# zharmad/SpinRelax

Measured on AMD Instinct MI355X. Metric: frame-vector-lag triples/s, C(t) + fit + R1/R2/NOE pipeline, higher is better.
Workload: dtype f32 transforms + f64 mean terms and chunk statistics (C(t): the reference's own type); f64 (histogram, fit, J(w), R1/R2/NOE)

## Files before the change

spinrelax_amd/csrc/sr_ct32.hip:

```cpp
#include "sr_internal.h"
#include "sr_ct32_fft.h"

namespace {

#ifndef SR_CT32_PF
#define SR_CT32_PF 0
#endif
#ifndef SR_CT32_NT
#define SR_CT32_NT 2
#endif
#ifndef SR_CT32_WAVES16
#define SR_CT32_WAVES16 3
#endif
#ifndef SR_CT32_WAVES
#define SR_CT32_WAVES 4
#endif
template <int N1, bool FULL>
__global__ __launch_bounds__(256, (N1 == 16 ? SR_CT32_WAVES16 : SR_CT32_WAVES)) void k_ct_rfft32(Ct32Args a)
{
    extern __shared__ __align__(16) unsigned char f32_smem[];
    c32 *lds = reinterpret_cast<c32 *>(f32_smem);
    constexpr int H = N1 * 256, M = 2 * H;
    constexpr int NZ = N1 == 4 ? 3 : (N1 == 8 ? 6 : (N1 == 12 ? 8 : 16));
    constexpr int IPT = N1 == 4 ? 3 : (N1 == 8 ? 6 : (N1 == 12 ? 8 : 11));
    c32 *tw1 = lds + rfft_img_slots(N1) + 256;
    c32 *tw3 = tw1 + 1024;
    float *aux = reinterpret_cast<float *>(tw3 + 256);
    const int tid0 = threadIdx.x;
    const int v = blockIdx.x / a.R, r = blockIdx.x - v * a.R;
    const int F = FULL ? 512 * NZ : a.F, L = FULL ? 256 * NZ : a.L;
    const int64_t start = a.chunk_start ? a.chunk_start[r] : (int64_t)r * F;
#ifdef SR_CT32_EXP_HOTLOADS
    const float *px = a.soa + (start & 1);
#else
    const float *px = a.soa + ((int64_t)v * 3 + 0) * a.Npad + start;
#endif
    const bool even = FULL || ((start | a.Npad | (int64_t)F) & 1) == 0;

#define SR_F32_LOAD1(DST, PLANE, T) SR_F32_LOADP(DST, PLANE, T, 0, NZ, 0)
#define SR_F32_LOADR(DST, PLANE, T, LO, HI) SR_F32_LOADP(DST, PLANE, T, LO, HI, 0)
#define SR_F32_LOAD1NT(DST, PLANE, T) SR_F32_LOADP(DST, PLANE, T, 0, NZ, SR_CT32_NT)
#define SR_F32_LOADP(DST, PLANE, T, LO, HI, POL)                                                 \
    {                                                                                            \
        const __amdgpu_buffer_rsrc_t rs_ = __builtin_amdgcn_make_buffer_rsrc(                    \
            const_cast<float *>(px + (int64_t)__builtin_amdgcn_readfirstlane(PLANE) * a.Npad), (short)0, F * 4, 0x00020000); \
        if (even) {                                                                              \
            _Pragma("unroll") for (int n1 = (LO); n1 < (HI); ++n1)                              \
                DST[n1] = __builtin_bit_cast(c32, __builtin_amdgcn_raw_buffer_load_b64(rs_, 8 * ((T) + 256 * n1), 0, (POL))); \
        } else {                                                                                 \
            _Pragma("unroll") for (int n1 = (LO); n1 < (HI); ++n1) {                            \
                const int ob_ = 8 * ((T) + 256 * n1);                                            \
                DST[n1] = c32{__builtin_bit_cast(float, __builtin_amdgcn_raw_buffer_load_b32(rs_, ob_, 0, (POL))),           \
                              __builtin_bit_cast(float, __builtin_amdgcn_raw_buffer_load_b32(rs_, ob_ + 4, 0, (POL)))};      \
            }                                                                                    \
        }                                                                                        \
    }
#define SR_F32_MASK(D0, D1, T, N1_)                                                              \
    if (!FULL) {                                                                                 \
        D0 = 2 * ((T) + 256 * (N1_)) < F ? D0 : 0.f;                                             \
        D1 = 2 * ((T) + 256 * (N1_)) + 1 < F ? D1 : 0.f;                                         \
    }
    {
        const int j = ((tid0 & 15) * (tid0 >> 4)) & 255;
        lds[rfft_img_slots(N1) + tid0] = c32{a.tab->w2[2 * j], a.tab->w2[2 * j + 1]};
#pragma unroll
        for (int jj = 0; jj < 4; ++jj) tw1[256 * jj + tid0] = c32{a.tab->w1[jj][2 * tid0], a.tab->w1[jj][2 * tid0 + 1]};
        tw3[tid0] = c32{a.tab->w3[2 * tid0], a.tab->w3[2 * tid0 + 1]};
        if (tid0 == 0) aux[50] = 0.f;
    }

    c32 sig[N1];
#pragma unroll
    for (int n1 = 0; n1 < N1; ++n1) sig[n1] = c32{0.f, 0.f};
    int nsig;
    {
        c32 xr[NZ], yr[NZ], zr[NZ];
        SR_F32_LOAD1(xr, 0, tid0)
        SR_F32_LOAD1(yr, 1, tid0)
        SR_F32_LOAD1NT(zr, 2, tid0)
        c32 s0 = {0.f, 0.f}, s1 = s0, s2 = s0, s3 = s0, s4 = s0, s5 = s0;
        float emax = 0.f;
#pragma unroll
        for (int n1 = 0; n1 < NZ; ++n1) {
            const c32 x = xr[n1], y = yr[n1], z = zr[n1];
            const c32 xx = x * x, yy = y * y, zz = z * z, q = xx + yy;
            s0 += (zz + zz) - q;
            s1 += xx - yy;
            s2 = pk_fma(x, y, s2);
            s3 = pk_fma(x, z, s3);
            s4 = pk_fma(y, z, s4);
            s5 += q + zz;
            c32 ev = (q + zz) - splat(1.0f);
            SR_F32_MASK(ev.x, ev.y, tid0, n1)
            emax = fmaxf(emax, fmaxf(fabsf(ev.x), fabsf(ev.y)));
        }
        const float t0 = wave_total_f32(s0.x + s0.y), t1 = wave_total_f32(s1.x + s1.y), t2 = wave_total_f32(s2.x + s2.y);
        const float t3 = wave_total_f32(s3.x + s3.y), t4 = wave_total_f32(s4.x + s4.y), t5 = wave_total_f32(s5.x + s5.y);
        emax = wave_max_f32(emax);
        if ((tid0 & 63) == 63) {
            float *o = aux + 8 * (tid0 >> 6);
            o[0] = t0; o[1] = t1; o[2] = t2; o[3] = t3; o[4] = t4; o[5] = t5; o[6] = emax;
        }
        __syncthreads();
        float m[6];
        const float invF = 1.0f / (float)F;
#pragma unroll
        for (int c = 0; c < 6; ++c)
            m[c] = __builtin_bit_cast(float, __builtin_amdgcn_readfirstlane(
                       __builtin_bit_cast(int, ((aux[c] + aux[8 + c]) + (aux[16 + c] + aux[24 + c])) * invF) & (int)0xFFFFFFF0));
        const float mx = fmaxf(fmaxf(aux[6], aux[14]), fmaxf(aux[22], aux[30]));
        const bool unit = __builtin_amdgcn_readfirstlane(mx < kUnitTolF ? 1 : 0) != 0;
        nsig = unit ? 5 : 6;
        const float wgt[6] = {1.0f, 3.0f, 12.0f, 12.0f, 12.0f, 2.0f};
        double Kc = unit ? 2.0 : 0.0;
#pragma unroll
        for (int c = 0; c < 6; ++c)
            if (c < 5 || !unit) Kc = fma((double)wgt[c] * (double)m[c], (double)m[c], Kc);
        if (tid0 == 0) {
#pragma unroll
            for (int c = 0; c < 6; ++c) {
                aux[32 + c] = m[c];
                aux[40 + c] = wgt[c] * m[c];
            }
            aux[48] = unit ? 2.0f : 0.f;
            *reinterpret_cast<double *>(aux + 52) = Kc;
        }
#pragma unroll
        for (int n1 = 0; n1 < NZ; ++n1) {
            c32 d = f32_sig0(xr[n1], yr[n1], zr[n1], m[0]);
            SR_F32_MASK(d.x, d.y, tid0, n1)
            sig[n1] = d;
        }
    }
    c32 W2[8];
#pragma unroll
    for (int q = 0; q < 8; ++q) W2[q] = c32{0.f, 0.f};
#ifdef SR_CT32_STAMPS
    long long stamp_acc[12] = {0, 0, 0, 0, 0, 0, 0, 0, 0, 0, 0, 0}, stamp_t = __builtin_amdgcn_s_memtime();
    const long long stamp_begin = stamp_t;
#define SR_STAMP_ARGS , stamp_acc, stamp_t
#else
#define SR_STAMP_ARGS
#endif
#pragma unroll 1
    for (int c = 0; c < nsig; ++c) {
        asm volatile("" ::: "memory");
        const int tid = opaque(tid0);
        const int k1 = (tid >> 4) & 15, k2a = tid & 15;
        const bool act = k1 < N1;
        const int pt = k1 != 0 ? (N1 - k1) * 16 + (15 - k2a) : (k2a != 0 ? 16 - k2a : 0);
        const int off0 = tid == 0 ? 1 : 0;
        const int cn = c + 1;
        c32 ar[NZ], br[NZ];
        if (SR_CT32_PF == 1 && cn < nsig) {
            SR_F32_LOAD1(ar, f32_plane_a(cn), tid)
            SR_F32_LOAD1(br, f32_plane_b(cn), tid)
        }
        c32 w[16];
        rfft32_workgroup<N1, true>(sig, w, lds, tw1, tid SR_STAMP_ARGS);
        SR_STAMP(6)
        if (SR_CT32_PF == 2 && cn < nsig) {
            SR_F32_LOAD1(ar, f32_plane_a(cn), tid)
            SR_F32_LOAD1(br, f32_plane_b(cn), tid)
        }
        SR_CT32_SYNC();
        SR_STAMP(7)
        if (act) {
            const float wgt = c == 0 ? 0.25f : (c == 1 ? 0.75f : (c == 5 ? 0.5f : 3.0f));
            const c32 *b = lds + 17 * pt + off0;
            const c32 wb = tw3[k1 + N1 * k2a];
#pragma unroll
            for (int q = 0; q < 8; q += 2) {
                const c32 zk0 = w[bitrev<4>(q)], zm0 = b[15 - q], zk1 = w[bitrev<4>(q + 1)], zm1 = b[14 - q];
                const c32 S0 = add_conj(zk0, zm0), S1 = add_conj(zk1, zm1);
                c32 T0 = sub_conj(zk0, zm0), T1 = sub_conj(zk1, zm1);
                cmulf2(T0, mulf_w32_rt(wb, q), T1, mulf_w32_rt(wb, q + 1));
                const c32 A0 = pair_re(S0, T0), B0 = pair_im(S0, T0), A1 = pair_re(S1, T1), B1 = pair_im(S1, T1);
                W2[q] = pk_fma(splat(wgt), pk_fma(A0, A0, B0 * B0), W2[q]);
                W2[q + 1] = pk_fma(splat(wgt), pk_fma(A1, A1, B1 * B1), W2[q + 1]);
            }
            if (off0) {
                const c32 zk = w[bitrev<4>(8)];
                const c32 D = {0.0f, 2.0f * zk.y};
                const c32 T = cmulf(D, mulf_w32_rt(wb, 8));
                const float pr = 2.0f * zk.x + T.y, pi = -T.x;
                aux[50] = fmaf(wgt, fmaf(pr, pr, pi * pi), aux[50]);
            }
        }
        SR_STAMP(8)
        if (cn < nsig) {
            asm volatile("" ::: "memory");
            const float mc = __builtin_bit_cast(float, __builtin_amdgcn_readfirstlane(__builtin_bit_cast(int, aux[32 + cn])));
#pragma unroll
            for (int g0 = 0; g0 < NZ; g0 += 8) {
                constexpr int GE = 8 < NZ ? 8 : NZ;
                if (g0 > 0) asm volatile("" ::: "memory");
                if (SR_CT32_PF == 0 || g0 > 0) {
                    if (SR_CT32_NT != 0 && cn == 3) {
                        SR_F32_LOADP(ar, 0, tid, g0, g0 + GE, SR_CT32_NT)
                    } else {
                        SR_F32_LOADR(ar, f32_plane_a(cn), tid, g0, g0 + GE)
                    }
                    if (SR_CT32_NT != 0 && cn == 2) {
                        SR_F32_LOADP(br, 1, tid, g0, g0 + GE, SR_CT32_NT)
                    } else {
                        SR_F32_LOADR(br, f32_plane_b(cn), tid, g0, g0 + GE)
                    }
                }
                if (cn == 1) {
#pragma unroll
                    for (int n1 = g0; n1 < g0 + GE; ++n1) ar[n1] = f32_sig1(ar[n1], br[n1], mc);
                } else if (cn == 5) {
                    c32 zr[NZ];
                    SR_F32_LOADR(zr, 2, tid, g0, g0 + GE)
#pragma unroll
                    for (int n1 = g0; n1 < g0 + GE; ++n1) ar[n1] = f32_sig5(ar[n1], br[n1], zr[n1], mc);
                } else {
#pragma unroll
                    for (int n1 = g0; n1 < g0 + GE; ++n1) ar[n1] = f32_sigp(ar[n1], br[n1], mc);
                }
#pragma unroll
                for (int n1 = g0; n1 < g0 + GE; ++n1) {
                    c32 d = ar[n1];
                    SR_F32_MASK(d.x, d.y, tid, n1)
                    sig[n1] = d;
                }
            }
#pragma unroll
            for (int n1 = NZ; n1 < N1; ++n1) sig[n1] = c32{0.f, 0.f};
        }
        SR_STAMP(9)
        SR_CT32_SYNC();
        SR_STAMP(10)
    }
#ifdef SR_CT32_STAMPS
    const long long stamp_loop_end = stamp_t;
#endif

    const int tid = opaque(tid0);
    const int k1 = (tid >> 4) & 15, k2a = tid & 15;
    const bool act = k1 < N1;
    const int pt = k1 != 0 ? (N1 - k1) * 16 + (15 - k2a) : (k2a != 0 ? 16 - k2a : 0);
    const int off0 = tid == 0 ? 1 : 0;
    if (act) {
        c32 *bk = lds + k1 + (N1 + 1) * k2a;
        c32 *bm = lds + (pt >> 4) + (N1 + 1) * (pt & 15) + 16 * (N1 + 1) * off0;
        const c32 wb = tw3[k1 + N1 * k2a];
#pragma unroll
        for (int q = 0; q < 8; ++q) {
            const float E = W2[q].x + W2[q].y, d = W2[q].x - W2[q].y;
            const c32 wk = mulf_w32_rt(wb, q);
            bk[16 * (N1 + 1) * q] = c32{fmaf(d, wk.y, E), d * wk.x};
            if (!(q == 0 && off0)) bm[16 * (N1 + 1) * (15 - q)] = c32{fmaf(-d, wk.y, E), d * wk.x};
        }
        if (off0) bk[16 * (N1 + 1) * 8] = c32{2.0f * aux[50], 0.0f};
    }
    __syncthreads();
    c32 w[16];
    {
        c32 yin[N1];
#pragma unroll
        for (int n1 = 0; n1 < N1; ++n1) {
            const int k = tid + 256 * n1;
            yin[n1] = lds[k + k / N1];
        }
        __syncthreads();
        rfft32_workgroup<N1, false>(yin, w, lds, tw1, tid SR_STAMP_ARGS);
    }
    __syncthreads();

    float *E = reinterpret_cast<float *>(lds);
    double *Tt = reinterpret_cast<double *>(lds);
    double *tot = reinterpret_cast<double *>(aux);
    {
        c32 xr[NZ], yr[NZ], zr[NZ];
        SR_F32_LOAD1NT(xr, 0, tid)
        SR_F32_LOAD1NT(yr, 1, tid)
        SR_F32_LOAD1NT(zr, 2, tid)
        float mm[6], wm[6];
#pragma unroll
        for (int c = 0; c < 6; ++c) {
            mm[c] = __builtin_bit_cast(float, __builtin_amdgcn_readfirstlane(__builtin_bit_cast(int, aux[32 + c])));
            wm[c] = __builtin_bit_cast(float, __builtin_amdgcn_readfirstlane(__builtin_bit_cast(int, aux[40 + c])));
        }
        const float weps = __builtin_bit_cast(float, __builtin_amdgcn_readfirstlane(__builtin_bit_cast(int, aux[48])));
        const bool unit = nsig == 5;
#pragma unroll
        for (int n1 = 0; n1 < NZ; ++n1) {
            const c32 x = xr[n1], y = yr[n1], z = zr[n1];
            c32 acc;
            if (unit) {
                acc.x = weps * (float)fma((double)x.x, (double)x.x, fma((double)y.x, (double)y.x, fma((double)z.x, (double)z.x, -1.0)));
                acc.y = weps * (float)fma((double)x.y, (double)x.y, fma((double)y.y, (double)y.y, fma((double)z.y, (double)z.y, -1.0)));
            } else {
                acc = splat(wm[5]) * f32_sig5(x, y, z, mm[5]);
            }
            acc = pk_fma(splat(wm[0]), f32_sig0(x, y, z, mm[0]), acc);
            acc = pk_fma(splat(wm[1]), f32_sig1(x, y, mm[1]), acc);
            acc = pk_fma(splat(wm[2]), f32_sigp(x, y, mm[2]), acc);
            acc = pk_fma(splat(wm[3]), f32_sigp(x, z, mm[3]), acc);
            acc = pk_fma(splat(wm[4]), f32_sigp(y, z, mm[4]), acc);
            SR_F32_MASK(acc.x, acc.y, tid, n1)
            *reinterpret_cast<c32 *>(E + 2 * (tid + 256 * n1)) = acc;
        }
    }
    __syncthreads();
    const int i0 = IPT * (255 - tid);
    double sfx[IPT], incl;
    {
        double hsum[IPT];
#pragma unroll
        for (int k = 0; k < IPT; ++k) {
            const int i = i0 + k, j = F - 1 - i;
            const float ei = E[min(i, F - 1)], ej = E[max(j, 0)];
            hsum[k] = (i <= j ? (double)ei : 0.0) + (i < j ? (double)ej : 0.0);
        }
        sfx[IPT - 1] = hsum[IPT - 1];
#pragma unroll
        for (int k = IPT - 2; k >= 0; --k) sfx[k] = hsum[k] + sfx[k + 1];
        incl = wave_scan_f64(sfx[0]);
        if ((tid & 63) == 63) tot[tid >> 6] = incl;
    }
    __syncthreads();
    {
        const int wave = tid >> 6;
        double off = incl - sfx[0];
#pragma unroll
        for (int w2 = 0; w2 < 3; ++w2) off += w2 < wave ? tot[w2] : 0.0;
        const double G0 = (tot[0] + tot[1]) + (tot[2] + tot[3]);
        const double Kc = *reinterpret_cast<const double *>(aux + 52);
#pragma unroll
        for (int k = 0; k < IPT; ++k) {
            const int d = i0 + k;
            if (d <= L) Tt[d] = fma((double)(F - d), Kc, G0 + (sfx[k] + off));
        }
        if (tid == 0 && L >= 256 * IPT) Tt[L] = fma((double)(F - L), Kc, G0);
    }
    __syncthreads();
    if (act) {
        double *out = a.psum + ((int64_t)v * a.R + r) * a.Lp;
        const double inv = 1.0 / (double)M, sixth = 1.0 / 6.0;
#pragma unroll
        for (int p = 0; p < 16; ++p) {
            const int m = k1 + N1 * (k2a + 16 * bitrev<4>(p));
            const int le = 2 * m, lod = 2 * m - 1;
            if (le >= 1 && le <= L) out[le] = fma((double)w[p].x, inv, Tt[le]) * sixth;
            if (lod >= 1 && lod <= L) out[lod] = fma((double)w[p].y, inv, Tt[lod]) * sixth;
        }
    }
#ifdef SR_CT32_STAMPS
    if ((tid & 63) == 0) {
        double *dbg = a.psum + ((int64_t)v * a.R + r) * a.Lp + L + 2 + 16 * (tid >> 6);
        for (int i = 0; i < 11; ++i) dbg[i] = (double)stamp_acc[i];
        dbg[11] = (double)(stamp_loop_end - stamp_begin);
        dbg[12] = (double)(__builtin_amdgcn_s_memtime() - stamp_begin);
    }
#endif
#undef SR_F32_LOAD1
#undef SR_F32_LOAD1NT
#undef SR_F32_LOADR
#undef SR_F32_LOADP
#undef SR_F32_MASK
}

template <int N1>
constexpr size_t f32_lds_bytes()
{
    return (size_t)(rfft_img_slots(N1) + 256 + 1024 + 256) * sizeof(c32) + 64 * sizeof(float);
}

template <int N1, bool FULL>
int launch_ct_rfft32_h(sr_ctx *ctx, const Ct32Args &a, int64_t series)
{
    size_t lds = f32_lds_bytes<N1>();
    static_assert(f32_lds_bytes<N1>() <= 64 * 1024, "k_ct_rfft32: the image is meant to fit the default LDS grant");
    if (ctx->ct_wg_per_cu > 0) {
        const size_t cap = ((size_t)160 * 1024 / (size_t)ctx->ct_wg_per_cu) & ~(size_t)1023;
        if (cap > lds && cap <= 64 * 1024) lds = cap;
    }
    constexpr size_t Fmax = N1 == 4 ? 1365 : (N1 == 8 ? 2730 : (N1 == 12 ? 4096 : 5461));
    static_assert((size_t)rfft_img_slots(N1) * sizeof(c32) >= (Fmax + 3) * 4, "k_ct_rfft32: E does not fit the image");
    static_assert((size_t)rfft_img_slots(N1) * sizeof(c32) >= (Fmax / 2 + 2) * 8, "k_ct_rfft32: Tt does not fit the image");
    return sr_launch(ctx, k_ct_rfft32<N1, FULL>, dim3((unsigned)series), dim3(256), lds, a);
}

}

const void *sr_ct32_tables(sr_ctx *ctx)
{
    Ct32Tab *tab = (Ct32Tab *)sr_workspace(ctx, SR_WS_FFT32, 4 * sizeof(Ct32Tab));
    if (!tab) return nullptr;
    if (!ctx->fft32_table_ready) {
        hipLaunchKernelGGL(k_ct32_init_table, dim3(4), dim3(256), 0, ctx->stream, tab);
        hipError_t e = hipGetLastError();
        if (e == hipSuccess) e = hipStreamSynchronize(ctx->stream);
        if (e != hipSuccess) { sr_set_error("k_ct32_init_table -> %s", hipGetErrorString(e)); return nullptr; }
        ctx->fft32_table_ready = 1;
    }
    return tab;
}

int sr_launch_ct_rfft32(sr_ctx *ctx, const sr_ct_job &j)
{
    const Ct32Tab *tab = (const Ct32Tab *)sr_ct32_tables(ctx);
    if (!tab) return -5;
    const int F = j.F;
    Ct32Args a;
    a.soa = j.soa; a.Npad = j.Npad; a.chunk_start = j.cs_dev; a.psum = j.psum;
    a.R = j.R; a.F = F; a.L = j.L; a.Lp = j.Lp;
    bool aligned = (j.Npad & 1) == 0 && (F & 1) == 0 && (((uintptr_t)j.soa) & 7) == 0;
    if (j.cs_host)
        for (int r = 0; r < j.R; ++r) aligned = aligned && (j.cs_host[r] & 1) == 0;
    const int need = F + j.L;
    SR_REQUIRE(need > 1024 && need <= 8192, -3, "k_ct_rfft32: F=%d outside the transform lengths", F);
    if (need <= 2048) {
        a.tab = tab + f32_tab_set(4);
        return launch_ct_rfft32_h<4, false>(ctx, a, j.series);
    }
    if (need <= 4096) {
        a.tab = tab + f32_tab_set(8);
        return launch_ct_rfft32_h<8, false>(ctx, a, j.series);
    }
    if (need <= 6144) {
        a.tab = tab + f32_tab_set(12);
        return aligned && F == 4096 ? launch_ct_rfft32_h<12, true>(ctx, a, j.series) : launch_ct_rfft32_h<12, false>(ctx, a, j.series);
    }
    a.tab = tab + f32_tab_set(16);
    return launch_ct_rfft32_h<16, false>(ctx, a, j.series);
}
```

spinrelax_amd/csrc/sr_ct32_fft.h:

```cpp
#pragma once
#include "sr_fft_common.h"

namespace {

typedef float c32 __attribute__((ext_vector_type(2)));
#define SR_PK __device__ __forceinline__
SR_PK c32 pk_fma(c32 a, c32 b, c32 c) { return __builtin_elementwise_fma(a, b, c); }
SR_PK c32 splat(float c) { return c32{c, c}; }
SR_PK c32 add_mi(c32 a, c32 b)
{
    c32 r;
    asm("v_pk_add_f32 %0, %1, %2 op_sel:[0,1] op_sel_hi:[1,0] neg_hi:[0,1]" : "=v"(r) : "v"(a), "v"(b));
    return r;
}
SR_PK c32 add_pi(c32 a, c32 b)
{
    c32 r;
    asm("v_pk_add_f32 %0, %1, %2 op_sel:[0,1] op_sel_hi:[1,0] neg_lo:[0,1]" : "=v"(r) : "v"(a), "v"(b));
    return r;
}
SR_PK c32 mi_sub(c32 a, c32 b)
{
    c32 r;
    asm("v_pk_add_f32 %0, %1, %2 op_sel:[1,1] op_sel_hi:[0,0] neg_lo:[0,1] neg_hi:[1,0]" : "=v"(r) : "v"(a), "v"(b));
    return r;
}
SR_PK c32 add_conj(c32 a, c32 b)
{
    c32 r;
    asm("v_pk_add_f32 %0, %1, %2 neg_hi:[0,1]" : "=v"(r) : "v"(a), "v"(b));
    return r;
}
SR_PK c32 sub_conj(c32 a, c32 b)
{
    c32 r;
    asm("v_pk_add_f32 %0, %1, %2 neg_lo:[0,1]" : "=v"(r) : "v"(a), "v"(b));
    return r;
}
SR_PK c32 pair_re(c32 s, c32 t)
{
    c32 r;
    asm("v_pk_add_f32 %0, %1, %2 op_sel:[0,1] op_sel_hi:[0,1] neg_hi:[0,1]" : "=v"(r) : "v"(s), "v"(t));
    return r;
}
SR_PK c32 pair_im(c32 s, c32 t)
{
    c32 r;
    asm("v_pk_add_f32 %0, %1, %2 op_sel:[1,0] op_sel_hi:[1,0] neg_lo:[0,1]" : "=v"(r) : "v"(s), "v"(t));
    return r;
}
SR_PK c32 cmulf(c32 a, c32 w)
{
    c32 t, r;
    asm("v_pk_mul_f32 %0, %1, %2 op_sel:[1,1] op_sel_hi:[1,0]" : "=v"(t) : "v"(a), "v"(w));
    asm("v_pk_fma_f32 %0, %1, %2, %3 op_sel:[0,0,0] op_sel_hi:[0,1,1] neg_lo:[0,0,1]" : "=v"(r) : "v"(a), "v"(w), "v"(t));
    return r;
}
SR_PK void cmulf2(c32 &a1, c32 w1, c32 &a2, c32 w2)
{
    c32 t1, t2;
    asm("v_pk_mul_f32 %2, %0, %4 op_sel:[1,1] op_sel_hi:[1,0]\n\t"
        "v_pk_mul_f32 %3, %1, %5 op_sel:[1,1] op_sel_hi:[1,0]\n\t"
        "v_pk_fma_f32 %0, %0, %4, %2 op_sel:[0,0,0] op_sel_hi:[0,1,1] neg_lo:[0,0,1]\n\t"
        "v_pk_fma_f32 %1, %1, %5, %3 op_sel:[0,0,0] op_sel_hi:[0,1,1] neg_lo:[0,0,1]"
        : "+v"(a1), "+v"(a2), "=&v"(t1), "=&v"(t2) : "v"(w1), "v"(w2));
}
template <int CBITS, int SBITS>
SR_PK c32 mul_const(c32 d)
{
    const float C = __builtin_bit_cast(float, CBITS), S = __builtin_bit_cast(float, SBITS);
    return pk_fma(d.yx, c32{S, -S}, d * splat(C));
}
constexpr int fbits(float f) { return __builtin_bit_cast(int, f); }

template <int E>
SR_PK c32 mulf_w32(c32 d)
{
    constexpr float c[16] = {1.0f, 0.9807852804032304f, 0.9238795325112867f, 0.8314696123025452f, 0.7071067811865476f,
                             0.5555702330196023f, 0.38268343236508984f, 0.19509032201612833f, 0.0f,
                             -0.1950903220161282f, -0.3826834323650897f, -0.555570233019602f, -0.7071067811865475f,
                             -0.8314696123025453f, -0.9238795325112867f, -0.9807852804032304f};
    constexpr float s[16] = {0.0f, 0.19509032201612825f, 0.3826834323650898f, 0.5555702330196022f, 0.7071067811865475f,
                             0.8314696123025452f, 0.9238795325112867f, 0.9807852804032304f, 1.0f, 0.9807852804032304f,
                             0.9238795325112867f, 0.8314696123025455f, 0.7071067811865476f, 0.5555702330196022f,
                             0.3826834323650899f, 0.1950903220161286f};
    if constexpr (E == 0) return d;
    else if constexpr (E == 8) return c32{d.y, -d.x};
    else if constexpr (E == 4) return add_mi(d, d) * splat(c[4]);
    else if constexpr (E == 12) return add_pi(d, d) * splat(-c[4]);
    else return mul_const<fbits(c[E]), fbits(s[E])>(d);
}
SR_PK c32 mulf_w32_rt(c32 d, int e)
{
    switch (e) {
        case 0: return mulf_w32<0>(d);
        case 1: return mulf_w32<1>(d);
        case 2: return mulf_w32<2>(d);
        case 3: return mulf_w32<3>(d);
        case 4: return mulf_w32<4>(d);
        case 5: return mulf_w32<5>(d);
        case 6: return mulf_w32<6>(d);
        case 7: return mulf_w32<7>(d);
        case 8: return mulf_w32<8>(d);
        case 9: return mulf_w32<9>(d);
        case 10: return mulf_w32<10>(d);
        case 11: return mulf_w32<11>(d);
        case 12: return mulf_w32<12>(d);
        case 13: return mulf_w32<13>(d);
        case 14: return mulf_w32<14>(d);
        default: return mulf_w32<15>(d);
    }
}
template <int E>
SR_PK c32 mulf_w24(c32 d)
{
    constexpr float c[15] = {1.0f, 0.9659258262890683f, 0.8660254037844387f, 0.7071067811865476f, 0.5000000000000001f,
                             0.25881904510252074f, 0.0f, -0.25881904510252063f, -0.4999999999999998f, -0.7071067811865475f,
                             -0.8660254037844387f, -0.9659258262890682f, -1.0f, -0.9659258262890683f, -0.8660254037844388f};
    constexpr float s[15] = {0.0f, 0.25881904510252074f, 0.49999999999999994f, 0.7071067811865475f, 0.8660254037844386f,
                             0.9659258262890683f, 1.0f, 0.9659258262890683f, 0.8660254037844387f, 0.7071067811865476f,
                             0.49999999999999994f, 0.258819045102521f, 0.0f, -0.2588190451025208f, -0.4999999999999997f};
    if constexpr (E == 0) return d;
    else if constexpr (E == 6) return c32{d.y, -d.x};
    else if constexpr (E == 12) return -d;
    else return mul_const<fbits(c[E]), fbits(s[E])>(d);
}

template <int LOGN, int S, int BLK, int J>
struct FftStageF {
    __device__ static __forceinline__ void run(c32 *v)
    {
        constexpr int N = 1 << LOGN;
        constexpr int half = N >> (S + 1);
        constexpr int i = BLK * 2 * half + J;
        constexpr int E = ((J << S) * (32 / N)) & 15;
        const c32 a = v[i], b = v[i + half];
        v[i] = a + b;
        if constexpr (E == 8) v[i + half] = mi_sub(a, b);
        else v[i + half] = mulf_w32<E>(a - b);
        if constexpr (J + 1 < half) FftStageF<LOGN, S, BLK, J + 1>::run(v);
        else if constexpr (BLK + 1 < (1 << S)) FftStageF<LOGN, S, BLK + 1, 0>::run(v);
        else if constexpr (S + 1 < LOGN) FftStageF<LOGN, S + 1, 0, 0>::run(v);
    }
};
template <int LOGN>
__device__ __forceinline__ void fftf_reg(c32 *v)
{
    FftStageF<LOGN, 0, 0, 0>::run(v);
}

template <int N1>
struct FStage1 : Stage1Map<N1> {
    __device__ static __forceinline__ void run(c32 *v) { fftf_reg<Stage1Map<N1>::LOG>(v); }
};
template <int B>
__device__ __forceinline__ void dft3f_col12(c32 *v, c32 (*y)[4])
{
    constexpr float h = 0.8660254037844386f;
    const c32 x0 = v[B], x1 = v[4 + B], x2 = v[8 + B];
    const c32 t = x1 + x2, d = x1 - x2;
    const c32 m = pk_fma(splat(-0.5f), t, x0);
    const c32 hd = d * splat(h);
    y[0][B] = x0 + t;
    y[1][B] = mulf_w24<2 * B>(add_mi(m, hd));
    y[2][B] = mulf_w24<4 * B>(add_pi(m, hd));
    if constexpr (B + 1 < 4) dft3f_col12<B + 1>(v, y);
}
template <>
struct FStage1<12> : Stage1Map<12> {
    __device__ static __forceinline__ void run(c32 *v)
    {
        c32 y[3][4];
        dft3f_col12<0>(v, y);
#pragma unroll
        for (int ka = 0; ka < 3; ++ka) {
            fftf_reg<2>(y[ka]);
#pragma unroll
            for (int q = 0; q < 4; ++q) v[4 * ka + q] = y[ka][q];
        }
    }
};

__device__ __forceinline__ c32 opaquef(c32 z)
{
    asm volatile("" : "+v"(z));
    return z;
}

template <int N, class KOF>
__device__ __forceinline__ void applyf_twiddles(c32 *v, const c32 *tw, int tid)
{
    c32 pw[16];
    pw[1] = opaquef(tw[tid]);
    pw[2] = opaquef(tw[256 + tid]);
    pw[4] = opaquef(tw[512 + tid]);
    pw[8] = opaquef(tw[768 + tid]);
    static_assert(N == 4 || N == 8 || N == 12 || N == 16, "the step-1 sizes");
    static_assert(KOF::k1(0) == 0, "entry 0 carries no twiddle");
    if constexpr (N == 4) {
        pw[3] = cmulf(pw[1], pw[2]);
        cmulf2(v[1], pw[2], v[2], pw[1]);
        v[3] = cmulf(v[3], pw[3]);
        return;
    } else if constexpr (N == 8) {
        pw[3] = pw[1]; pw[5] = pw[1];
        cmulf2(pw[3], pw[2], pw[5], pw[4]);
        pw[6] = pw[2]; pw[7] = pw[3];
        cmulf2(pw[6], pw[4], pw[7], pw[4]);
        v[1] = cmulf(v[1], pw[4]);
#pragma unroll
        for (int p = 2; p + 1 < N; p += 2) cmulf2(v[p], pw[KOF::k1(p)], v[p + 1], pw[KOF::k1(p + 1)]);
        return;
    }
    pw[3] = pw[1]; pw[5] = pw[1]; pw[6] = pw[2]; pw[9] = pw[1]; pw[10] = pw[2];
    cmulf2(pw[3], pw[2], pw[5], pw[4]);
    cmulf2(pw[6], pw[4], pw[9], pw[8]);
    pw[7] = pw[3]; pw[11] = pw[3];
    if constexpr (N == 12) {
        cmulf2(pw[10], pw[8], pw[7], pw[4]);
        cmulf2(pw[11], pw[8], v[1], pw[KOF::k1(1)]);
    } else {
        pw[12] = pw[4];
        cmulf2(pw[10], pw[8], pw[12], pw[8]);
        pw[13] = pw[5]; pw[14] = pw[6];
        cmulf2(pw[7], pw[4], pw[11], pw[8]);
        cmulf2(pw[13], pw[8], pw[14], pw[8]);
        pw[15] = pw[7];
        cmulf2(pw[15], pw[8], v[1], pw[KOF::k1(1)]);
    }
#pragma unroll
    for (int p = 2; p + 1 < N; p += 2) cmulf2(v[p], pw[KOF::k1(p)], v[p + 1], pw[KOF::k1(p + 1)]);
}

struct Ct32Tab {
    float w1[4][2 * 256];
    float w2[2 * 256];
    float w3[2 * 256];
};
__host__ __device__ constexpr int f32_tab_set(int N1) { return N1 / 4 - 1; }
__global__ void k_ct32_init_table(Ct32Tab *tab)
{
    const int t = threadIdx.x, set = blockIdx.x;
    const double H = 1024.0 * (double)(set + 1);
    double sn, cs;
    for (int j = 0; j < 4; ++j) {
        const int e = (t << j) % (int)H;
        sincospi(2.0 * (double)e / H, &sn, &cs);
        tab[set].w1[j][2 * t] = (float)cs;
        tab[set].w1[j][2 * t + 1] = (float)-sn;
    }
    sincospi(2.0 * (double)t / 256.0, &sn, &cs);
    tab[set].w2[2 * t] = (float)cs;
    tab[set].w2[2 * t + 1] = (float)-sn;
    sincospi((double)t / H, &sn, &cs);
    tab[set].w3[2 * t] = (float)cs;
    tab[set].w3[2 * t + 1] = (float)-sn;
}

struct Ct32Args {
    const float *soa;
    int64_t Npad;
    const int64_t *chunk_start;
    const Ct32Tab *tab;
    double *psum;
    int R, F, L, Lp;
};

#ifdef SR_CT32_STAMPS
#define SR_STAMP(I) { const long long t_ = __builtin_amdgcn_s_memtime(); stamp_acc[I] += t_ - stamp_t; stamp_t = t_; }
#else
#define SR_STAMP(I)
#endif
#ifdef SR_CT32_EXP_NOBAR
#define SR_CT32_SYNC() __builtin_amdgcn_wave_barrier()
#else
#define SR_CT32_SYNC() __syncthreads()
#endif

template <int N1, bool SPECTRUM>
__device__ __forceinline__ void rfft32_workgroup(c32 *v, c32 *w, c32 *lds, const c32 *tw1, int tid
#ifdef SR_CT32_STAMPS
                                                 , long long *stamp_acc, long long &stamp_t
#endif
)
{
    FStage1<N1>::run(v);
    applyf_twiddles<N1, FStage1<N1>>(v, tw1, tid);
    {
        c32 *b = lds + tid + (tid >> 4);
#pragma unroll
        for (int p = 0; p < N1; ++p) b[272 * FStage1<N1>::k1(p)] = v[p];
    }
    SR_STAMP(0)
    SR_CT32_SYNC();
    SR_STAMP(1)
    const int k1 = tid >> 4, lo = tid & 15;
    const bool act = k1 < N1;
    if (act) {
        c32 u[16];
        const c32 *b = lds + 272 * k1 + lo;
#pragma unroll
        for (int h = 0; h < 16; ++h) u[h] = b[17 * h];
#ifdef SR_CT32_STAMPS
        asm volatile("s_waitcnt lgkmcnt(0)" ::: "memory");
        SR_STAMP(2)
#endif
        fftf_reg<4>(u);
        {
            const c32 *tw = lds + rfft_img_slots(N1) + lo;
#pragma unroll
            for (int p = 1; p < 15; p += 2) cmulf2(u[p], tw[16 * bitrev<4>(p)], u[p + 1], tw[16 * bitrev<4>(p + 1)]);
            u[15] = cmulf(u[15], tw[16 * bitrev<4>(15)]);
        }
        c32 *bw = lds + 272 * k1 + lo;
#pragma unroll
        for (int p = 0; p < 16; ++p) bw[17 * bitrev<4>(p)] = u[p];
        SR_STAMP(3)
    }
    __builtin_amdgcn_fence(__ATOMIC_RELEASE, "wavefront");
    __builtin_amdgcn_wave_barrier();
    __builtin_amdgcn_fence(__ATOMIC_ACQUIRE, "wavefront");
    if (act) {
        const c32 *b = lds + 17 * tid;
#pragma unroll
        for (int e = 0; e < 16; ++e) w[e] = b[e];
#ifdef SR_CT32_STAMPS
        asm volatile("s_waitcnt lgkmcnt(0)" ::: "memory");
        SR_STAMP(4)
#endif
        fftf_reg<4>(w);
        SR_STAMP(5)
        if (SPECTRUM) {
            c32 *bo = lds + 17 * tid;
#pragma unroll
            for (int p = 0; p < 16; ++p)
                if (bitrev<4>(p) >= 8) bo[bitrev<4>(p)] = w[p];
            if (tid == 0) bo[16] = w[0];
        }
    }
}

constexpr float kUnitTolF = 5e-7f;

__device__ __forceinline__ int f32_plane_a(int c) { return c == 4 ? 1 : 0; }
__device__ __forceinline__ int f32_plane_b(int c) { return c == 3 || c == 4 ? 2 : 1; }

SR_PK c32 f32_sig0(c32 x, c32 y, c32 z, float m) { return pk_fma(z + z, z, -pk_fma(x, x, pk_fma(y, y, splat(m)))); }
SR_PK c32 f32_sig1(c32 x, c32 y, float m) { return pk_fma(x, x, -pk_fma(y, y, splat(m))); }
SR_PK c32 f32_sigp(c32 a, c32 b, float m) { return pk_fma(a, b, splat(-m)); }
SR_PK c32 f32_sig5(c32 x, c32 y, c32 z, float m) { return pk_fma(z, z, pk_fma(x, x, pk_fma(y, y, splat(-m)))); }

}
```

spinrelax_amd/csrc/sr_ct_long.h:

```cpp
#pragma once
#include "sr_internal.h"
#include "sr_ct32_fft.h"

namespace {

constexpr int kB = 4096;
constexpr int kH = 4096;
constexpr int kSpecLen = 4160;
constexpr int kKTile = 64;

struct CtlConst {
    float m[6];
    float wm[6];
    float weps;
    int nsig;
    double Kc;
    double G0;
};

struct CtlArgs {
    const float *soa;
    int64_t Npad;
    const int64_t *chunk_start;
    CtlConst *consts;
    double *psum;
    const Ct32Tab *tab;
    c32 *spec;
    double2 *Q;
    const double2 *itab;
    int R, F, L, Lp, nb, nd;
    int s0;
};

__device__ __forceinline__ float uniform_f(float v)
{
    return __builtin_bit_cast(float, __builtin_amdgcn_readfirstlane(__builtin_bit_cast(int, v)));
}

__global__ __launch_bounds__(256) void k_ctl_consts(CtlArgs a)
{
    __shared__ float red[4][8];
    const int tid = threadIdx.x, s = blockIdx.x;
    const int v = s / a.R, r = s - v * a.R, F = a.F;
    const int64_t start = a.chunk_start ? a.chunk_start[r] : (int64_t)r * F;
    const float *px = a.soa + (int64_t)v * 3 * a.Npad + start, *py = px + a.Npad, *pz = py + a.Npad;
    float s0 = 0.f, s1 = 0.f, s2 = 0.f, s3 = 0.f, s4 = 0.f, s5 = 0.f, emax = 0.f;
    for (int j = tid; j < F; j += 256) {
        const float x = px[j], y = py[j], z = pz[j];
        const float xx = x * x, yy = y * y, zz = z * z, q = xx + yy;
        s0 += (zz + zz) - q;
        s1 += xx - yy;
        s2 = fmaf(x, y, s2);
        s3 = fmaf(x, z, s3);
        s4 = fmaf(y, z, s4);
        s5 += q + zz;
        emax = fmaxf(emax, fabsf((q + zz) - 1.0f));
    }
    s0 = wave_total_f32(s0); s1 = wave_total_f32(s1); s2 = wave_total_f32(s2);
    s3 = wave_total_f32(s3); s4 = wave_total_f32(s4); s5 = wave_total_f32(s5);
    emax = wave_max_f32(emax);
    if ((tid & 63) == 63) {
        float *o = red[tid >> 6];
        o[0] = s0; o[1] = s1; o[2] = s2; o[3] = s3; o[4] = s4; o[5] = s5; o[6] = emax;
    }
    __syncthreads();
    if (tid == 0) {
        const float wgt[6] = {1.0f, 3.0f, 12.0f, 12.0f, 12.0f, 2.0f};
        const float invF = 1.0f / (float)F;
        const bool unit = fmaxf(fmaxf(red[0][6], red[1][6]), fmaxf(red[2][6], red[3][6])) < kUnitTolF;
        CtlConst c;
        double Kc = unit ? 2.0 : 0.0;
        for (int i = 0; i < 6; ++i) {
            const float mean = ((red[0][i] + red[1][i]) + (red[2][i] + red[3][i])) * invF;
            c.m[i] = __builtin_bit_cast(float, __builtin_bit_cast(int, mean) & (int)0xFFFFFFF0);
            c.wm[i] = wgt[i] * c.m[i];
            if (i < 5 || !unit) Kc = fma((double)wgt[i] * (double)c.m[i], (double)c.m[i], Kc);
        }
        c.weps = unit ? 2.0f : 0.f;
        c.nsig = unit ? 5 : 6;
        c.Kc = Kc;
        c.G0 = 0.0;
        a.consts[s] = c;
    }
}

__device__ __forceinline__ void ctl_load(c32 *dst, const float *plane, int Fb, bool even, int tid)
{
    const __amdgpu_buffer_rsrc_t rs = __builtin_amdgcn_make_buffer_rsrc(const_cast<float *>(plane), (short)0, Fb * 4, 0x00020000);
    if (even) {
#pragma unroll
        for (int n1 = 0; n1 < 8; ++n1)
            dst[n1] = __builtin_bit_cast(c32, __builtin_amdgcn_raw_buffer_load_b64(rs, 8 * (tid + 256 * n1), 0, 0));
    } else {
#pragma unroll
        for (int n1 = 0; n1 < 8; ++n1) {
            const int ob = 8 * (tid + 256 * n1);
            dst[n1] = c32{__builtin_bit_cast(float, __builtin_amdgcn_raw_buffer_load_b32(rs, ob, 0, 0)),
                          __builtin_bit_cast(float, __builtin_amdgcn_raw_buffer_load_b32(rs, ob + 4, 0, 0))};
        }
    }
}

constexpr size_t ctl_spectra_lds_bytes() { return (size_t)(rfft_img_slots(16) + 256 + 1024 + 256) * sizeof(c32); }

__global__ __launch_bounds__(256, 3) void k_ctl_spectra(CtlArgs a)
{
    extern __shared__ __align__(16) unsigned char ctl_smem[];
    c32 *lds = reinterpret_cast<c32 *>(ctl_smem);
    constexpr int N1 = 16, NZ = 8;
    c32 *tw1 = lds + rfft_img_slots(N1) + 256;
    c32 *tw3 = tw1 + 1024;
    const int tid0 = threadIdx.x, blk = blockIdx.x, sl = blockIdx.y, s = a.s0 + sl;
    const int v = s / a.R, r = s - v * a.R;
    const int64_t start = (a.chunk_start ? a.chunk_start[r] : (int64_t)r * a.F) + (int64_t)blk * kB;
    const int Fb = min(kB, a.F - blk * kB);
    const float *px = a.soa + (int64_t)v * 3 * a.Npad + start;
    const bool even = ((start | a.Npad | (int64_t)Fb) & 1) == 0;
    {
        const int j = ((tid0 & 15) * (tid0 >> 4)) & 255;
        lds[rfft_img_slots(N1) + tid0] = c32{a.tab->w2[2 * j], a.tab->w2[2 * j + 1]};
#pragma unroll
        for (int jj = 0; jj < 4; ++jj) tw1[256 * jj + tid0] = c32{a.tab->w1[jj][2 * tid0], a.tab->w1[jj][2 * tid0 + 1]};
        tw3[tid0] = c32{a.tab->w3[2 * tid0], a.tab->w3[2 * tid0 + 1]};
    }
    const CtlConst *cc = a.consts + s;
    const int nsig = __builtin_amdgcn_readfirstlane(cc->nsig);
    __syncthreads();
#pragma unroll 1
    for (int c = 0; c < nsig; ++c) {
        asm volatile("" ::: "memory");
        const int tid = opaque(tid0);
        const float mc = uniform_f(cc->m[c]);
        c32 sig[N1];
        {
            c32 ar[NZ], br[NZ];
            ctl_load(ar, px + (int64_t)__builtin_amdgcn_readfirstlane(f32_plane_a(c)) * a.Npad, Fb, even, tid);
            ctl_load(br, px + (int64_t)__builtin_amdgcn_readfirstlane(f32_plane_b(c)) * a.Npad, Fb, even, tid);
            if (c == 0 || c == 5) {
                c32 zr[NZ];
                ctl_load(zr, px + 2 * a.Npad, Fb, even, tid);
#pragma unroll
                for (int n1 = 0; n1 < NZ; ++n1) ar[n1] = c == 0 ? f32_sig0(ar[n1], br[n1], zr[n1], mc) : f32_sig5(ar[n1], br[n1], zr[n1], mc);
            } else if (c == 1) {
#pragma unroll
                for (int n1 = 0; n1 < NZ; ++n1) ar[n1] = f32_sig1(ar[n1], br[n1], mc);
            } else {
#pragma unroll
                for (int n1 = 0; n1 < NZ; ++n1) ar[n1] = f32_sigp(ar[n1], br[n1], mc);
            }
#pragma unroll
            for (int n1 = 0; n1 < NZ; ++n1) {
                c32 d = ar[n1];
                d.x = 2 * (tid + 256 * n1) < Fb ? d.x : 0.f;
                d.y = 2 * (tid + 256 * n1) + 1 < Fb ? d.y : 0.f;
                sig[n1] = d;
            }
#pragma unroll
            for (int n1 = NZ; n1 < N1; ++n1) sig[n1] = c32{0.f, 0.f};
        }
        c32 w[16];
        rfft32_workgroup<N1, true>(sig, w, lds, tw1, tid);
        __syncthreads();
        const int k1 = (tid >> 4) & 15, k2a = tid & 15;
        const int pt = k1 != 0 ? (N1 - k1) * 16 + (15 - k2a) : (k2a != 0 ? 16 - k2a : 0);
        const int off0 = tid == 0 ? 1 : 0;
        const c32 *b = lds + 17 * pt + off0;
        const c32 wb = tw3[k1 + N1 * k2a];
        c32 *out = a.spec + ((int64_t)(sl * 6 + c) * a.nb + blk) * kSpecLen + tid;
#pragma unroll
        for (int q = 0; q < 8; q += 2) {
            const c32 zk0 = w[bitrev<4>(q)], zm0 = b[15 - q], zk1 = w[bitrev<4>(q + 1)], zm1 = b[14 - q];
            const c32 S0 = add_conj(zk0, zm0), S1 = add_conj(zk1, zm1);
            c32 T0 = sub_conj(zk0, zm0), T1 = sub_conj(zk1, zm1);
            cmulf2(T0, mulf_w32_rt(wb, q), T1, mulf_w32_rt(wb, q + 1));
            const c32 A0 = pair_re(S0, T0), B0 = pair_im(S0, T0), A1 = pair_re(S1, T1), B1 = pair_im(S1, T1);
            out[256 * q] = c32{A0.x, B0.x};
            out[2048 + 256 * q] = c32{A0.y, -B0.y};
            out[256 * (q + 1)] = c32{A1.x, B1.x};
            out[2048 + 256 * (q + 1)] = c32{A1.y, -B1.y};
        }
        if (off0) {
            const c32 zk = w[bitrev<4>(8)];
            const c32 D = {0.0f, 2.0f * zk.y};
            const c32 T = cmulf(D, mulf_w32_rt(wb, 8));
            out[4096] = c32{2.0f * zk.x + T.y, -T.x};
        }
        __syncthreads();
    }
}

__global__ void k_ctl_init_table(double2 *tab)
{
    const int e = blockIdx.x * 256 + threadIdx.x;
    double sn, cs;
    sincospi((double)e / 4096.0, &sn, &cs);
    tab[e] = double2{cs, sn};
}

__device__ __forceinline__ double2 cmul64(double2 a, double2 b) { return double2{fma(a.x, b.x, -a.y * b.y), fma(a.x, b.y, a.y * b.x)}; }

__global__ __launch_bounds__(256) void k_ctl_inverse(CtlArgs a)
{
    extern __shared__ __align__(16) unsigned char ctl_smem[];
    double2 *lds = reinterpret_cast<double2 *>(ctl_smem);
    const int tid = threadIdx.x, d = blockIdx.x, sl = blockIdx.y, s = a.s0 + sl;
    const double2 *Q = a.Q + ((int64_t)sl * a.nd + d) * kSpecLen;
    const double2 *T = a.itab;
#pragma unroll 2
    for (int q = 0; q < 8; ++q) {
        const int k = (tid >> 4) + 16 * ((tid & 15) + 16 * q);
        const double2 P = Q[256 * q + tid], Pm = Q[2048 + 256 * q + tid];
        const double2 S = {P.x + Pm.x, P.y - Pm.y}, D = {P.x - Pm.x, P.y + Pm.y};
        const double2 td = cmul64(T[k], D);
        const double2 U = {-td.y, td.x};
        lds[k] = double2{S.x + U.x, S.y + U.y};
        if (k != 0) lds[kH - k] = double2{S.x - U.x, -(S.y - U.y)};
    }
    if (tid == 0) {
        const double2 P = Q[4096];
        lds[kH / 2] = double2{2.0 * P.x, -2.0 * P.y};
    }
    for (int st = 0; st < 8; ++st) {
        __syncthreads();
        const int lh = 11 - st, half = 1 << lh;
#pragma unroll 2
        for (int n = 0; n < 8; ++n) {
            const int bf = tid + 256 * n, jj = bf & (half - 1), i0 = ((bf >> lh) << (lh + 1)) + jj, i1 = i0 + half;
            const double2 A = lds[i0], Bv = lds[i1];
            lds[i0] = double2{A.x + Bv.x, A.y + Bv.y};
            lds[i1] = cmul64(double2{A.x - Bv.x, A.y - Bv.y}, T[(jj << st) << 1]);
        }
    }
    __syncthreads();
    double2 u[16];
#pragma unroll
    for (int p = 0; p < 16; ++p) u[p] = lds[16 * tid + p];
    {
        constexpr double cs16[8] = {1.0, 0.9238795325112867, 0.7071067811865476, 0.3826834323650898, 0.0,
                                    -0.3826834323650898, -0.7071067811865476, -0.9238795325112867};
        constexpr double sn16[8] = {0.0, 0.3826834323650898, 0.7071067811865476, 0.9238795325112867, 1.0,
                                    0.9238795325112867, 0.7071067811865476, 0.3826834323650898};
#pragma unroll
        for (int st = 0; st < 4; ++st) {
            const int half = 8 >> st;
#pragma unroll
            for (int bf = 0; bf < 8; ++bf) {
                const int jj = bf & (half - 1), i0 = ((bf / half) * 2 * half) + jj, i1 = i0 + half, e = jj << st;
                const double2 A = u[i0], Bv = u[i1];
                u[i0] = double2{A.x + Bv.x, A.y + Bv.y};
                u[i1] = cmul64(double2{A.x - Bv.x, A.y - Bv.y}, double2{cs16[e], sn16[e]});
            }
        }
    }
    __syncthreads();
    double *lag = reinterpret_cast<double *>(ctl_smem);
    {
        const int n0 = (int)(__builtin_bitreverse32((unsigned)tid) >> 24);
#pragma unroll
        for (int p = 0; p < 16; p += 2) {
            const int n = 256 * bitrev<4>(p) + n0;
            lag[2 * n] = u[p].x;
            lag[2 * n + 1] = u[p].y;
        }
    }
    __syncthreads();
    double *out = a.psum + (int64_t)s * a.Lp;
    const double G0 = a.consts[s].G0, inv = 1.0 / 8192.0, sixth = 1.0 / 6.0;
#pragma unroll 4
    for (int i = 0; i < 16; ++i) {
        const int m = tid + 256 * i, D = d * kB + m;
        if (D >= 1 && D <= a.L) out[D] = fma(lag[m], inv, out[D] + G0) * sixth;
    }
}

inline int64_t ctl_spec_bytes(int64_t F) { return 6 * ((F + kB - 1) / kB) * kSpecLen * (int64_t)sizeof(c32); }
inline int64_t ctl_q_bytes(int64_t F) { return ((F / 2) / kB + 1) * kSpecLen * (int64_t)sizeof(double2); }

inline int ctl_tables(sr_ctx *ctx, const Ct32Tab **tab32, const double2 **itab_out)
{
    const Ct32Tab *t = (const Ct32Tab *)sr_ct32_tables(ctx);
    if (!t) return -5;
    double2 *itab = (double2 *)sr_workspace(ctx, SR_WS_CTLONG_TAB, (size_t)kH * sizeof(double2));
    if (!itab) return -5;
    if (!ctx->ctlong_table_ready) {
        hipLaunchKernelGGL(k_ctl_init_table, dim3(kH / 256), dim3(256), 0, ctx->stream, itab);
        SR_HIP(hipGetLastError());
        SR_HIP(hipStreamSynchronize(ctx->stream));
        ctx->ctlong_table_ready = 1;
    }
    *tab32 = t + f32_tab_set(16);
    *itab_out = itab;
    return 0;
}

inline int ctl_acquire(sr_ctx *ctx, size_t bytes, unsigned char **ws)
{
    if (!ctx->ctlong_ev) SR_HIP(hipEventCreateWithFlags(&ctx->ctlong_ev, hipEventDisableTiming));
    *ws = (unsigned char *)sr_workspace(ctx, SR_WS_CTLONG, bytes);
    if (!*ws) return -5;
    if (ctx->ctlong_ev_set) SR_HIP(hipStreamWaitEvent(ctx->stream, ctx->ctlong_ev, 0));
    return 0;
}
inline int ctl_release(sr_ctx *ctx)
{
    SR_HIP(hipEventRecord(ctx->ctlong_ev, ctx->stream));
    ctx->ctlong_ev_set = 1;
    return 0;
}

constexpr size_t kCtlInverseLds = (size_t)kH * sizeof(double2);
static_assert(ctl_spectra_lds_bytes() <= 64 * 1024, "k_ctl_spectra: the image is meant to fit the default LDS grant");

}
```

Measured before the change: 59150 billion.

## Use 64-bit LDS loads, permute tw3 table, and pad Tt to avoid bank conflicts

Complex values in LDS are now read through a 64-bit relaxed atomic load helper, so the compiler emits single ds_read_b64 loads instead of split 32-bit loads or reordered accesses. The tw3 twiddle table is stored permuted so each thread reads tw3[tid] contiguously, where before it used a strided index. The f64 Tt array gets a padding slot every 8 entries to reduce LDS bank conflicts, and the static size check is updated to match. The cost is a larger Tt footprint. Using atomics to steer codegen may also limit the compiler's scheduling.

Result: faster. 59870 billion (median of 6 runs) (+1.2%).

```diff
diff --git a/spinrelax_amd/csrc/sr_ct32.hip b/spinrelax_amd/csrc/sr_ct32.hip
--- a/spinrelax_amd/csrc/sr_ct32.hip
+++ b/spinrelax_amd/csrc/sr_ct32.hip
@@ -15,6 +15,8 @@
 #ifndef SR_CT32_WAVES
 #define SR_CT32_WAVES 4
 #endif
+__device__ __forceinline__ int f32_tt_slot(int d) { return d + (d >> 3); }
+
 template <int N1, bool FULL>
 __global__ __launch_bounds__(256, (N1 == 16 ? SR_CT32_WAVES16 : SR_CT32_WAVES)) void k_ct_rfft32(Ct32Args a)
 {
@@ -65,7 +67,10 @@
         lds[rfft_img_slots(N1) + tid0] = c32{a.tab->w2[2 * j], a.tab->w2[2 * j + 1]};
 #pragma unroll
         for (int jj = 0; jj < 4; ++jj) tw1[256 * jj + tid0] = c32{a.tab->w1[jj][2 * tid0], a.tab->w1[jj][2 * tid0 + 1]};
-        tw3[tid0] = c32{a.tab->w3[2 * tid0], a.tab->w3[2 * tid0 + 1]};
+        {
+            const int t3 = (tid0 >> 4) + N1 * (tid0 & 15);
+            tw3[tid0] = c32{a.tab->w3[2 * t3], a.tab->w3[2 * t3 + 1]};
+        }
         if (tid0 == 0) aux[50] = 0.f;
     }
 
@@ -168,10 +173,10 @@
         if (act) {
             const float wgt = c == 0 ? 0.25f : (c == 1 ? 0.75f : (c == 5 ? 0.5f : 3.0f));
             const c32 *b = lds + 17 * pt + off0;
-            const c32 wb = tw3[k1 + N1 * k2a];
+            const c32 wb = lds_ld64(tw3 + tid);
 #pragma unroll
             for (int q = 0; q < 8; q += 2) {
-                const c32 zk0 = w[bitrev<4>(q)], zm0 = b[15 - q], zk1 = w[bitrev<4>(q + 1)], zm1 = b[14 - q];
+                const c32 zk0 = w[bitrev<4>(q)], zm0 = lds_ld64(b + 15 - q), zk1 = w[bitrev<4>(q + 1)], zm1 = lds_ld64(b + 14 - q);
                 const c32 S0 = add_conj(zk0, zm0), S1 = add_conj(zk1, zm1);
                 c32 T0 = sub_conj(zk0, zm0), T1 = sub_conj(zk1, zm1);
                 cmulf2(T0, mulf_w32_rt(wb, q), T1, mulf_w32_rt(wb, q + 1));
@@ -245,7 +250,7 @@
     if (act) {
         c32 *bk = lds + k1 + (N1 + 1) * k2a;
         c32 *bm = lds + (pt >> 4) + (N1 + 1) * (pt & 15) + 16 * (N1 + 1) * off0;
-        const c32 wb = tw3[k1 + N1 * k2a];
+        const c32 wb = lds_ld64(tw3 + tid);
 #pragma unroll
         for (int q = 0; q < 8; ++q) {
             const float E = W2[q].x + W2[q].y, d = W2[q].x - W2[q].y;
@@ -262,7 +267,7 @@
 #pragma unroll
         for (int n1 = 0; n1 < N1; ++n1) {
             const int k = tid + 256 * n1;
-            yin[n1] = lds[k + k / N1];
+            yin[n1] = lds_ld64(lds + k + k / N1);
         }
         __syncthreads();
         rfft32_workgroup<N1, false>(yin, w, lds, tw1, tid SR_STAMP_ARGS);
@@ -332,9 +337,9 @@
 #pragma unroll
         for (int k = 0; k < IPT; ++k) {
             const int d = i0 + k;
-            if (d <= L) Tt[d] = fma((double)(F - d), Kc, G0 + (sfx[k] + off));
-        }
-        if (tid == 0 && L >= 256 * IPT) Tt[L] = fma((double)(F - L), Kc, G0);
+            if (d <= L) Tt[f32_tt_slot(d)] = fma((double)(F - d), Kc, G0 + (sfx[k] + off));
+        }
+        if (tid == 0 && L >= 256 * IPT) Tt[f32_tt_slot(L)] = fma((double)(F - L), Kc, G0);
     }
     __syncthreads();
     if (act) {
@@ -344,8 +349,8 @@
         for (int p = 0; p < 16; ++p) {
             const int m = k1 + N1 * (k2a + 16 * bitrev<4>(p));
             const int le = 2 * m, lod = 2 * m - 1;
-            if (le >= 1 && le <= L) out[le] = fma((double)w[p].x, inv, Tt[le]) * sixth;
-            if (lod >= 1 && lod <= L) out[lod] = fma((double)w[p].y, inv, Tt[lod]) * sixth;
+            if (le >= 1 && le <= L) out[le] = fma((double)w[p].x, inv, lds_ld64(Tt + f32_tt_slot(le))) * sixth;
+            if (lod >= 1 && lod <= L) out[lod] = fma((double)w[p].y, inv, lds_ld64(Tt + f32_tt_slot(lod))) * sixth;
         }
     }
 #ifdef SR_CT32_STAMPS
@@ -380,7 +385,7 @@
     }
     constexpr size_t Fmax = N1 == 4 ? 1365 : (N1 == 8 ? 2730 : (N1 == 12 ? 4096 : 5461));
     static_assert((size_t)rfft_img_slots(N1) * sizeof(c32) >= (Fmax + 3) * 4, "k_ct_rfft32: E does not fit the image");
-    static_assert((size_t)rfft_img_slots(N1) * sizeof(c32) >= (Fmax / 2 + 2) * 8, "k_ct_rfft32: Tt does not fit the image");
+    static_assert((size_t)rfft_img_slots(N1) * sizeof(c32) >= (Fmax / 2 + Fmax / 16 + 2) * 8, "k_ct_rfft32: Tt does not fit the image");
     return sr_launch(ctx, k_ct_rfft32<N1, FULL>, dim3((unsigned)series), dim3(256), lds, a);
 }
 
diff --git a/spinrelax_amd/csrc/sr_ct32_fft.h b/spinrelax_amd/csrc/sr_ct32_fft.h
--- a/spinrelax_amd/csrc/sr_ct32_fft.h
+++ b/spinrelax_amd/csrc/sr_ct32_fft.h
@@ -181,6 +181,15 @@
     }
 };
 
+SR_PK c32 lds_ld64(const c32 *p)
+{
+    return __builtin_bit_cast(c32, __hip_atomic_load(reinterpret_cast<const unsigned long long *>(p), __ATOMIC_RELAXED, __HIP_MEMORY_SCOPE_WAVEFRONT));
+}
+SR_PK double lds_ld64(const double *p)
+{
+    return __builtin_bit_cast(double, __hip_atomic_load(reinterpret_cast<const unsigned long long *>(p), __ATOMIC_RELAXED, __HIP_MEMORY_SCOPE_WAVEFRONT));
+}
+
 __device__ __forceinline__ c32 opaquef(c32 z)
 {
     asm volatile("" : "+v"(z));
@@ -191,10 +200,11 @@
 __device__ __forceinline__ void applyf_twiddles(c32 *v, const c32 *tw, int tid)
 {
     c32 pw[16];
-    pw[1] = opaquef(tw[tid]);
-    pw[2] = opaquef(tw[256 + tid]);
-    pw[4] = opaquef(tw[512 + tid]);
-    pw[8] = opaquef(tw[768 + tid]);
+    const c32 b1 = lds_ld64(tw + tid), b2 = lds_ld64(tw + 256 + tid), b4 = lds_ld64(tw + 512 + tid), b8 = lds_ld64(tw + 768 + tid);
+    pw[1] = opaquef(b1);
+    pw[2] = opaquef(b2);
+    pw[4] = opaquef(b4);
+    pw[8] = opaquef(b8);
     static_assert(N == 4 || N == 8 || N == 12 || N == 16, "the step-1 sizes");
     static_assert(KOF::k1(0) == 0, "entry 0 carries no twiddle");
     if constexpr (N == 4) {
@@ -300,7 +310,7 @@
         c32 u[16];
         const c32 *b = lds + 272 * k1 + lo;
 #pragma unroll
-        for (int h = 0; h < 16; ++h) u[h] = b[17 * h];
+        for (int h = 0; h < 16; ++h) u[h] = lds_ld64(b + 17 * h);
 #ifdef SR_CT32_STAMPS
         asm volatile("s_waitcnt lgkmcnt(0)" ::: "memory");
         SR_STAMP(2)
@@ -309,8 +319,8 @@
         {
             const c32 *tw = lds + rfft_img_slots(N1) + lo;
 #pragma unroll
-            for (int p = 1; p < 15; p += 2) cmulf2(u[p], tw[16 * bitrev<4>(p)], u[p + 1], tw[16 * bitrev<4>(p + 1)]);
-            u[15] = cmulf(u[15], tw[16 * bitrev<4>(15)]);
+            for (int p = 1; p < 15; p += 2) cmulf2(u[p], lds_ld64(tw + 16 * bitrev<4>(p)), u[p + 1], lds_ld64(tw + 16 * bitrev<4>(p + 1)));
+            u[15] = cmulf(u[15], lds_ld64(tw + 16 * bitrev<4>(15)));
         }
         c32 *bw = lds + 272 * k1 + lo;
 #pragma unroll
@@ -323,7 +333,7 @@
     if (act) {
         const c32 *b = lds + 17 * tid;
 #pragma unroll
-        for (int e = 0; e < 16; ++e) w[e] = b[e];
+        for (int e = 0; e < 16; ++e) w[e] = lds_ld64(b + e);
 #ifdef SR_CT32_STAMPS
         asm volatile("s_waitcnt lgkmcnt(0)" ::: "memory");
         SR_STAMP(4)
diff --git a/spinrelax_amd/csrc/sr_ct_long.h b/spinrelax_amd/csrc/sr_ct_long.h
--- a/spinrelax_amd/csrc/sr_ct_long.h
+++ b/spinrelax_amd/csrc/sr_ct_long.h
@@ -121,7 +121,10 @@
         lds[rfft_img_slots(N1) + tid0] = c32{a.tab->w2[2 * j], a.tab->w2[2 * j + 1]};
 #pragma unroll
         for (int jj = 0; jj < 4; ++jj) tw1[256 * jj + tid0] = c32{a.tab->w1[jj][2 * tid0], a.tab->w1[jj][2 * tid0 + 1]};
-        tw3[tid0] = c32{a.tab->w3[2 * tid0], a.tab->w3[2 * tid0 + 1]};
+        {
+            const int t3 = (tid0 >> 4) + N1 * (tid0 & 15);
+            tw3[tid0] = c32{a.tab->w3[2 * t3], a.tab->w3[2 * t3 + 1]};
+        }
     }
     const CtlConst *cc = a.consts + s;
     const int nsig = __builtin_amdgcn_readfirstlane(cc->nsig);
@@ -165,11 +168,11 @@
         const int pt = k1 != 0 ? (N1 - k1) * 16 + (15 - k2a) : (k2a != 0 ? 16 - k2a : 0);
         const int off0 = tid == 0 ? 1 : 0;
         const c32 *b = lds + 17 * pt + off0;
-        const c32 wb = tw3[k1 + N1 * k2a];
+        const c32 wb = lds_ld64(tw3 + tid);
         c32 *out = a.spec + ((int64_t)(sl * 6 + c) * a.nb + blk) * kSpecLen + tid;
 #pragma unroll
         for (int q = 0; q < 8; q += 2) {
-            const c32 zk0 = w[bitrev<4>(q)], zm0 = b[15 - q], zk1 = w[bitrev<4>(q + 1)], zm1 = b[14 - q];
+            const c32 zk0 = w[bitrev<4>(q)], zm0 = lds_ld64(b + 15 - q), zk1 = w[bitrev<4>(q + 1)], zm1 = lds_ld64(b + 14 - q);
             const c32 S0 = add_conj(zk0, zm0), S1 = add_conj(zk1, zm1);
             c32 T0 = sub_conj(zk0, zm0), T1 = sub_conj(zk1, zm1);
             cmulf2(T0, mulf_w32_rt(wb, q), T1, mulf_w32_rt(wb, q + 1));
```
